# MIMUW-RL/space-gym

Measured on AMD Instinct MI355X. Metric: env-steps/sec at batch=65536, GoalContinuous3P-v0, 1/2/4/8 MI355X, higher is better.
Workload: dtype f32

## Files before the change

space_gym_amd/csrc/sg_device.hpp:

```cpp
#ifndef SG_DEVICE_HPP
#define SG_DEVICE_HPP

#include <math.h>
#include <stdint.h>

#include "sg_config.h"

#if defined(__HIPCC__)
#define SG_FN __device__ __forceinline__
#define SG_MFN __device__ __forceinline__
#else
#define SG_FN static inline
#define SG_MFN inline
#endif

#ifndef SG_STAMP
#define SG_STAMP(slot)
#endif

namespace sg {

#if defined(__HIP_DEVICE_COMPILE__)
SG_FN float rsq(float x) { return __builtin_amdgcn_rsqf(x); }
SG_FN float rcp(float x) { return __builtin_amdgcn_rcpf(x); }
// ... 925 lines not shown

SG_FN void tile_center(const SgDev &c, const Tiling &T, uint32_t tile, float &x, float &y) {
    uint32_t row = (tile * c.t_cols_rcp16) >> 16, col = tile - row * (uint32_t)c.t_cols;
    const float shift = (col == 1u) ? T.cs1 : (col == 2u) ? T.cs2 : (col == 3u) ? T.cs3 : T.cs0;
    float tx = c.t_x0 + (float)col * 1.5f * c.t_a + shift;
    float y0 = T.case_b ? c.t_y0 - 0.5f * c.t_hex_h : c.t_y0;
    float ycol = (col & 1u) ? 0.5f * c.t_hex_h : 0.0f;
    float ty = y0 - (float)row * c.t_hex_h + (T.case_b ? ycol : -ycol);
    x = T.flip ? ty : tx;
    y = T.flip ? tx : ty;
}

SG_FN void disc_in_tile(const SgDev &c, const Tiling &T, uint32_t tile, float noise_radius, uint32_t w, float &x, float &y) {
    float s, co;
    sincos_acc(kTwoPi * u16(w >> 16), s, co);
    float r = noise_radius * fsqrt(u16(w));
    tile_center(c, T, tile, x, y);
    x = fmaf(r, co, x);
    y = fmaf(r, s, y);
}

SG_FN void choose_goal_tile(const SgDev &c, Tiling &T, bool first, const uint32_t (&w)[4]) {
    if (!first) {
        T.free_counts = free_add(T.free_counts, T.ship_tile);
        T.ship_tile = T.goal_tile;
    }
    if ((w[0] & 0xffu) < 64u) {
        T.goal_tile = T.ship_tile;
    } else {
        const uint32_t n = free_total(T.free_counts), n_cand = n < 3u ? n : 3u;
        const uint32_t cols = (uint32_t)c.t_cols, sr = (T.ship_tile * c.t_cols_rcp16) >> 16, sc = T.ship_tile - sr * cols;
        const uint32_t draws[3] = {w[1] >> 16, w[1], w[2] >> 16};
        uint32_t chosen[3] = {0u, 0u, 0u};
        const uint32_t j0 = below16(draws[0], n);
        chosen[0] = j0;
        const uint32_t v1_old = (j0 == 1u) ? 0u : 1u;
        uint32_t j1 = 0xffffffffu;
        if (n_cand > 1) {
            j1 = 1u + below16(draws[1], n - 1u);
            chosen[1] = (j1 == j0) ? 0u : j1;
        }
        if (n_cand > 2) {
            const uint32_t j2 = 2u + below16(draws[2], n - 2u);
            chosen[2] = (j2 == j1) ? v1_old : (j2 == j0) ? 0u : j2;
        }
        uint32_t best_tile = 0;
        int best_dist = -1;
        const FreePrefix fp = free_prefix(T.free_counts);
#pragma unroll
        for (uint32_t i = 0; i < 3; i++) {
            if (i < n_cand) {
                uint32_t tile = free_at(fp, chosen[i]);
                uint32_t r = (tile * c.t_cols_rcp16) >> 16, cc = tile - r * cols;
                int dist = abs((int)r - (int)sr) + abs((int)cc - (int)sc);
                if (dist > best_dist) { best_dist = dist; best_tile = tile; }
            }
        }
        T.goal_tile = best_tile;
        T.free_counts = free_remove(T.free_counts, best_tile);
    }
}

SG_FN void choose_goal(const SgDev &c, Tiling &T, bool first, const uint32_t (&w)[4], float &gx, float &gy) {
    choose_goal_tile(c, T, first, w);
    disc_in_tile(c, T, T.goal_tile, c.noise_goal, w[3], gx, gy);
}

SG_FN void box_muller(uint32_t w1, uint32_t w2, float &z0, float &z1) {
    float r = fsqrt(-2.0f * 0.6931471805599453f * flog2(u23(w1)));
    float s, co;
    sincos_acc(kTwoPi * u23(w2), s, co);
    z0 = r * co;
    z1 = r * s;
}

struct ShipInit { float x, y, th, vx, vy, om; };

SG_FN void layout_from_words(const SgDev &c, uint32_t flags, uint32_t c01, uint32_t c23, Tiling &T) {
    T.case_b = flags & 1u; T.flip = (flags >> 1) & 1u;
    const float a0 = u16(c01 >> 16), a1 = a0 + u16(c01);
    const float a2 = (c.t_cols > 2) ? a1 + u16(c23 >> 16) : a1, a3 = (c.t_cols > 3) ? a2 + u16(c23) : a2;
    const float k = c.t_free_x * rcp(a3);
    T.cs0 = a0 * k; T.cs1 = a1 * k;
    T.cs2 = (c.t_cols > 2) ? a2 * k : 0.0f; T.cs3 = (c.t_cols > 3) ? a3 * k : 0.0f;
}

template <int N>
SG_FN void tiles_from_words(const SgDev &c, uint32_t flags, uint32_t t01, uint32_t t23, uint32_t t45, Tiling &T,
                            uint32_t (&tiles)[N + 1]) {
    const uint32_t draws[6] = {t01 >> 16, t01, t23 >> 16, t23, t45 >> 16, t45};
    uint64_t perm = 0xfedcba9876543210ull;
    const uint32_t nt = (uint32_t)c.t_tiles;
#pragma unroll
    for (uint32_t i = 0; i <= (uint32_t)N; i++) {
        uint32_t j = i + below16(draws[i], nt - i);
        uint64_t vi = (perm >> (4 * i)) & 15ull, vj = (perm >> (4 * j)) & 15ull;
        perm = (perm & ~((15ull << (4 * i)) | (15ull << (4 * j)))) | (vj << (4 * i)) | (vi << (4 * j));
        tiles[i] = (uint32_t)vj;
    }
    if (N == 2 && ((flags >> 8) & 0xffu) < 64u) {
        const uint32_t d = (flags >> 16) & 3u;
        tiles[0] = (d == 0) ? 1u : (d == 1) ? 2u : (d == 2) ? 0u : 3u;
        tiles[1] = (d < 2) ? 0u : 1u;
        tiles[2] = (d < 2) ? 3u : 2u;
    }
    uint64_t used = 0;
#pragma unroll
    for (int i = 0; i <= N; i++) used |= 1ull << (4 * tiles[i]);
    const uint64_t all = (nt >= 16u) ? 0x1111111111111111ull : (0x1111111111111111ull & ((1ull << (4 * nt)) - 1ull));
    T.free_counts = all & ~used;
    T.ship_tile = tiles[0];
}

SG_FN void kinematics_from_words(const SgDev &c, uint32_t wth, uint32_t b0, uint32_t b1, uint32_t b2, uint32_t b3, ShipInit &s) {
    s.th = kTwoPi * u23(wth);
    float z0, z1, z2, z3;
    box_muller(b0, b1, z0, z1);
    box_muller(b2, b3, z2, z3);
    s.vx = z0 * c.vel_std; s.vy = z1 * c.vel_std;
    s.om = fminf(fmaxf(z2 * c.omega_std, -c.omega_max), c.omega_max);
}

template <int N>
SG_FN void goal_reset(const SgDev &c, uint32_t env_global, Tiling &T, ShipInit &s, float (&px)[N], float (&py)[N],
                      float &gx, float &gy) {
    uint32_t w[4 * kGoalResetBlocks];
#pragma unroll
    for (uint32_t b = 0; b < (uint32_t)kGoalResetBlocks; b++) {
        uint32_t o[4];
        philox4x32_10(c.seed_lo, c.seed_hi, env_global, T.episode, b, kStreamReset, o);
        w[4 * b] = o[0]; w[4 * b + 1] = o[1]; w[4 * b + 2] = o[2]; w[4 * b + 3] = o[3];
    }
    T.goal_draws = 0;
    const uint32_t flags = w[0];
    layout_from_words(c, flags, w[1], w[2], T);
    uint32_t tiles[N + 1];
    tiles_from_words<N>(c, flags, w[3], w[4], w[5], T, tiles);
    disc_in_tile(c, T, tiles[0], c.noise_ship, w[8], s.x, s.y);
#pragma unroll
    for (int j = 0; j < N; j++) disc_in_tile(c, T, tiles[j + 1], c.noise_planet, w[9 + j], px[j], py[j]);
    const uint32_t gw[4] = {flags >> 24, w[6], w[7], w[13]};
    T.goal_tile = 0xffu;
    choose_goal(c, T, true, gw, gx, gy);
    kinematics_from_words(c, w[14], w[16], w[17], w[18], w[19], s);
}

SG_FN void goal_resample(const SgDev &c, uint32_t env_global, Tiling &T, float &gx, float &gy) {
    uint32_t w[4];
    T.goal_draws += 1;
    philox4x32_10(c.seed_lo, c.seed_hi, env_global, T.episode, T.goal_draws, kStreamGoal, w);
    choose_goal(c, T, false, w, gx, gy);
}

SG_FN void kepler_reset(const SgDev &c, uint32_t env_global, uint32_t episode, ShipInit &s, float &phi, float &ecc) {
    uint32_t w[4 * kKeplerResetBlocks];
#pragma unroll
    for (uint32_t b = 0; b < (uint32_t)kKeplerResetBlocks; b++) {
        uint32_t o[4];
        philox4x32_10(c.seed_lo, c.seed_hi, env_global, episode, b, kStreamReset, o);
        w[4 * b] = o[0]; w[4 * b + 1] = o[1]; w[4 * b + 2] = o[2]; w[4 * b + 3] = o[3];
    }
    float sa, ca;
    sincos_acc(kTwoPi * u23(w[0]), sa, ca);
    float dist = fmaf(c.kep_rmax - c.kep_rmin, u23(w[1]), c.kep_rmin);
    s.x = ca * dist; s.y = sa * dist;
    if (c.randomize_orbit) { ecc = u23(w[3]) * 0.7f; phi = u23(w[4]) * kTwoPi; }
    kinematics_from_words(c, w[2], w[8], w[9], w[10], w[11], s);
}

SG_FN void random_action_words(uint32_t seed_lo, uint32_t seed_hi, uint32_t env_global, uint64_t step, uint32_t &w0, uint32_t &w1) {
    uint32_t o[4];
    const uint64_t p = step >> 1;
    philox4x32_10(seed_lo, seed_hi, env_global, (uint32_t)p, (uint32_t)(p >> 32), kStreamAction, o);
    w0 = (step & 1u) ? o[2] : o[0];
    w1 = (step & 1u) ? o[3] : o[1];
}

template <int N>
struct GoalEnv {
    float x, y, th, vx, vy, om;
    float gx, gy;
    float px[N], py[N];
};
struct KeplerEnv {
    float x, y, th, vx, vy, om;
    float phi, ecc;
};

SG_FN void translate_action(float &a0, float &a1, float max_engine_force, float &engine, float &F, float &om) {
    a0 = fminf(fmaxf(a0, -1.0f), 1.0f);
    a1 = fminf(fmaxf(a1, -1.0f), 1.0f);
    engine = (a0 + 1.0f) * 0.5f;
    F = engine * max_engine_force;
    om = a1 * 5.0f;
}

template <bool ACCEL>
SG_FN void steering(const SgDev &c, float a1, float om_cmd, float om_state, float &om0, float &alpha) {
    if (ACCEL && c.steering_acceleration) { om0 = om_state; alpha = (a1 * c.max_thruster_force) * c.inv_moi; }
    else { om0 = om_cmd; alpha = 0.0f; }
}

SG_FN void load_action(bool discrete, const void *actions, int64_t idx, float &a0, float &a1) {
    if (discrete) {
        const int k = static_cast<const int32_t *>(actions)[idx];
        const bool engine = (k == 1) | (k == 4) | (k == 5);
        a0 = engine ? 1.0f : -1.0f;
        a1 = (k == 2 || k == 4) ? -1.0f : (k == 3 || k == 5) ? 1.0f : 0.0f;
    } else {
        const float *p = static_cast<const float *>(actions) + 2 * idx;
        a0 = p[0]; a1 = p[1];
    }
}

template <int N, typename CFG>
SG_FN void goal_observe(const CFG &c, const GoalEnv<N> &e, float (&obs)[7 + 2 * N + 2]) {
    float s, co;
    sincos_acc(e.th, s, co);
    obs[0] = e.x; obs[1] = e.y; obs[2] = co; obs[3] = s; obs[4] = e.vx; obs[5] = e.vy; obs[6] = e.om;
#pragma unroll
    for (int j = 0; j < N; j++) lidar(e.px[j] - e.x, e.py[j] - e.y, c.planet_r, c.two_over_world, obs[7 + 2 * j], obs[8 + 2 * j]);
    obs[7 + 2 * N] = (e.gx - e.x) * c.two_over_world;
    obs[8 + 2 * N] = (e.gy - e.y) * c.two_over_world;
}

template <typename CFG>
SG_FN void kepler_observe(const CFG &c, const KeplerEnv &e, float (&obs)[10]) {
    float s, co;
    sincos_acc(e.th, s, co);
    obs[0] = e.x; obs[1] = e.y; obs[2] = co; obs[3] = s; obs[4] = e.vx; obs[5] = e.vy; obs[6] = e.om;
    obs[7] = c.randomize_orbit ? e.phi : (float)c.k_phi;
    obs[8] = c.randomize_orbit ? e.ecc : (float)c.k_ecc;
    obs[9] = (float)c.k_a;
}

template <int N, bool ACCEL = false>
SG_FN void goal_env_begin(const SgDev &c, const GoalEnv<N> &e, float a0, float a1, Integrator<N, N, true, ACCEL> &I,
                          bool use_probe = true) {
    float engine, F, om, om0, alpha;
    translate_action(a0, a1, c.max_engine_force, engine, F, om);
    steering<ACCEL>(c, a1, om, e.om, om0, alpha);
    float cR[N];
    double cRd[N];
#pragma unroll
    for (int j = 0; j < N; j++) { cR[j] = c.planet_r; cRd[j] = c.planet_r_d; }
    I.begin(c.h, c.half_world, c.gm, F, om0, alpha, c.omega_limit, e.x, e.y, e.th, e.vx, e.vy, e.px, e.py, cR, cRd, use_probe);
}

struct GoalStepConsts {
    double goal_r2, danger_r2, survival, goal_scale, safety_scale, sparse;
    float planet_r, two_over_world;
};
SG_FN GoalStepConsts goal_step_consts(const SgDev &c) {
    GoalStepConsts k;
    k.goal_r2 = c.goal_r2; k.danger_r2 = c.danger_r2; k.survival = c.survival; k.goal_scale = c.goal_scale;
    k.safety_scale = c.safety_scale; k.sparse = c.sparse; k.planet_r = c.planet_r; k.two_over_world = c.two_over_world;
    return k;
}

struct KeplerStepConsts {
    double k_gm, k_C, k_Cr, k_phi, k_ecc, k_a;
    float k_Ca;
    int32_t randomize_orbit;
};
SG_FN KeplerStepConsts kepler_step_consts(const SgDev &c) {
    KeplerStepConsts k;
    k.k_gm = c.k_gm; k.k_C = c.k_C; k.k_Cr = c.k_Cr; k.k_phi = c.k_phi; k.k_ecc = c.k_ecc; k.k_a = c.k_a; k.k_Ca = c.k_Ca;
    k.randomize_orbit = c.randomize_orbit;
    return k;
}

struct GoalRewardProfile {
    double danger_r2, survival, goal_scale, safety_scale, sparse;
};
struct KeplerRewardProfile {
    double k_C, k_Cr;
    float k_Ca;
};
struct GoalRewardView {
    double goal_r2, danger_r2, survival, goal_scale, safety_scale, sparse;
};
SG_FN GoalRewardView goal_reward_view(const SgDev &c, const GoalRewardProfile &p) {
    GoalRewardView v;
    v.goal_r2 = c.goal_r2; v.danger_r2 = p.danger_r2; v.survival = p.survival; v.goal_scale = p.goal_scale;
    v.safety_scale = p.safety_scale; v.sparse = p.sparse;
    return v;
}
struct KeplerRewardView {
    double k_gm, k_C, k_Cr;
    float k_Ca;
};
SG_FN KeplerRewardView kepler_reward_view(const SgDev &c, const KeplerRewardProfile &p) {
    KeplerRewardView v;
    v.k_gm = c.k_gm; v.k_C = p.k_C; v.k_Cr = p.k_Cr; v.k_Ca = p.k_Ca;
    return v;
}

struct StepConsts {
    float max_engine_force, h, half_world, gm, omega_limit, planet_r, max_thruster_force, inv_moi;
    double planet_r_d;
    int32_t steering_acceleration;
};
SG_FN StepConsts step_consts(const SgDev &c) {
    StepConsts k;
    k.max_engine_force = c.max_engine_force; k.h = c.h; k.half_world = c.half_world; k.gm = c.gm; k.omega_limit = c.omega_limit;
    k.planet_r = c.planet_r; k.max_thruster_force = c.max_thruster_force; k.inv_moi = c.inv_moi; k.planet_r_d = c.planet_r_d;
// ... 98 lines not shown
```

space_gym_amd/csrc/sg_engine.hip:

```cpp
#include <hip/hip_runtime.h>
#include <hip/hip_ext.h>

#include <algorithm>
#include <array>
#include <cmath>
#include <cstdarg>
#include <cstdio>
#include <cstdlib>
#include <cstring>
#include <limits>
#include <new>
#include <string>
#include <tuple>
#include <type_traits>
#include <utility>
#include <vector>

#include "../../include/spacegym.h"

#ifdef SG_STAMPS
constexpr int kStampSlots = 16, kStampWaves = 4096;
__device__ unsigned long long sg_dbg_stamps[kStampSlots * kStampWaves];
#ifdef SG_STAMPS_ACC_ONLY
#define SG_STAMP(slot)
// ... 613 lines not shown
    using Env = GoalEnv<N>;
    using Rec = StepRecord<N>;
    using Integ = Integrator<N, N, true, ACCEL>;
    static constexpr int D = 7 + 2 * N + 2;
    static constexpr int kPre = 320, kWordsAt = 256;
    static constexpr bool kResample = true;
    static constexpr bool kTouchParams = true, kFinishAction = false;
    __device__ __forceinline__ explicit GoalStep(const SgDev &) {}
    __device__ __forceinline__ void load(const SgBuffers &b, int jj, float4 *base) const {
        __builtin_amdgcn_global_load_lds((gbl_void *)(b.pl[0] + jj), (lds_void *)(base + 128), 16, 0, 0);
        if constexpr (N > 2) __builtin_amdgcn_global_load_lds((gbl_void *)(b.pl[1] + jj), (lds_void *)(base + 192), 16, 0, 0);
    }
    __device__ __forceinline__ void read(const float4 *blk, int lane, Env &e) const {
        const float4 q0 = blk[lane], q1 = blk[64 + lane], p0 = blk[128 + lane];
        float4 p1 = {};
        if constexpr (N > 2) p1 = blk[192 + lane];
        e.x = q0.x; e.y = q0.y; e.th = q0.z; e.vx = q0.w;
        e.vy = q1.x; e.om = q1.y; e.gx = q1.z; e.gy = q1.w;
        e.px[0] = p0.x; e.py[0] = p0.y; e.px[1] = p0.z; e.py[1] = p0.w;
        if constexpr (N > 2) { e.px[2] = p1.x; e.py[2] = p1.y; }
        if constexpr (N > 3) { e.px[3] = p1.z; e.py[3] = p1.w; }
    }
    __device__ __forceinline__ static float2 q1_hi(const Env &e) { return make_float2(e.gx, e.gy); }
    __device__ __forceinline__ static int first(const SgDev &c, const Env &e, float2 a, StepResult &sr) {
        Integ I;
        goal_env_begin<N, ACCEL>(c, e, a.x, a.y, I);
        return I.first(sr, []() __attribute__((always_inline)) -> bool { return true; });
    }
    __device__ __forceinline__ static void integrate(const SgDev &c, const Env &e, float2 a, StepResult &sr) {
        Integ I;
        goal_env_begin<N, ACCEL>(c, e, a.x, a.y, I);
        I.run(sr);
    }
    __device__ __forceinline__ static void load_env(const SgBuffers &b, int i, Env &e) { load_goal_env<N>(b, i, e); }
    struct Ready {};
    __device__ __forceinline__ Ready load_finisher(const SgDev &, const SgBuffers &, int, const Env &) const { return {}; }
    __device__ __forceinline__ int pair_finish(const SgDev &c, const SgBuffers &b, Ready, Env &e, float2 a, const PairHand &h, bool live,
                                               float (&o)[D], float &r) const {
        return pair_finish_r(c, c, b, Ready{}, e, a, h, live, o, r);
    }
    template <typename RC>
    __device__ __forceinline__ static int pair_finish_r(const SgDev &c, const RC &rc, const SgBuffers &b, Ready, Env &e, float2,
                                                        const PairHand &h, bool live, float (&o)[D], float &r) {
        int hit;
        r = goal_reward<N>(rc, e.x, e.y, h.dXd, h.dYd, e.px, e.py, e.gx, e.gy, hit);
        e.x = (float)((double)e.x + h.dXd); e.y = (float)((double)e.y + h.dYd);
        e.th = h.th; e.vx = h.vx; e.vy = h.vy; e.om = h.om;
        goal_observe<N>(c, e, o);
        count_hits(b.cnt, live && hit);
        return hit;
    }
    __device__ __forceinline__ int finish(const SgDev &c, const SgBuffers &b, int, Env &e, float2, const StepResult &sr, bool kept,
                                          float (&o)[D], float &r) const {
        int dn, hit;
        goal_env_finish<N>(c, e, sr, o, r, dn, hit);
        count_hits(b.cnt, kept && hit);
        return hit;
    }
    template <typename RC>
    __device__ __forceinline__ static int finish_r(const SgDev &c, const RC &rc, const SgBuffers &b, Env &e, float2, const StepResult &sr,
                                                   bool kept, float (&o)[D], float &r) {
        int dn, hit;
        goal_env_finish_r<N>(c, rc, e, sr, o, r, dn, hit);
        count_hits(b.cnt, kept && hit);
        return hit;
    }
    __device__ __forceinline__ int replay(const SgDev &c, const SgBuffers &b, int, Env &e, float2 a, bool terminal, bool have,
                                          float (&o)[D], float &r, int &dn) const {
        StepResult r2;
        {
            Integ I;
            goal_env_begin<N, ACCEL>(c, e, a.x, a.y, I, false);
            I.run(r2);
        }
        if (terminal) r2.done = 1;
        int hit;
        goal_env_finish<N>(c, e, r2, o, r, dn, hit);
        count_hits(b.cnt, have && hit);
        return hit;
    }
    template <typename RC>
    __device__ __forceinline__ static int replay_r(const SgDev &c, const RC &rc, const SgBuffers &b, Env &e, float2 a, bool terminal,
                                                   bool have, float (&o)[D], float &r, int &dn) {
        StepResult r2;
        {
            Integ I;
            goal_env_begin<N, ACCEL>(c, e, a.x, a.y, I, false);
            I.run(r2);
        }
        if (terminal) r2.done = 1;
        int hit;
        goal_env_finish_r<N>(c, rc, e, r2, o, r, dn, hit);
        count_hits(b.cnt, have && hit);
        return hit;
    }
    struct Next {
        Tiling T;
        ShipInit s;
        float px[N], py[N], gx, gy;
    };
    __device__ __forceinline__ static float2 kept_orbit(const SgBuffers &, int) { return make_float2(0.0f, 0.0f); }
    __device__ __forceinline__ static float2 reset_orbit(const SgDev &) { return make_float2(0.0f, 0.0f); }
    __device__ __forceinline__ static void next(const SgDev &c, int env, uint32_t episode, float2, Next &n) {
        n.T.episode = episode;
        goal_reset<N>(c, c.env_index_base + (uint32_t)env, n.T, n.s, n.px, n.py, n.gx, n.gy);
    }
    __device__ __forceinline__ void install(const SgDev &c, const SgBuffers &b, int env, uint32_t episode, const Next &n, Env &e,
                                            float (&o)[D]) const {
        e.x = n.s.x; e.y = n.s.y; e.th = n.s.th; e.vx = n.s.vx; e.vy = n.s.vy; e.om = n.s.om; e.gx = n.gx; e.gy = n.gy;
#pragma unroll
        for (int j = 0; j < N; j++) { e.px[j] = n.px[j]; e.py[j] = n.py[j]; }
        store_goal_ship<N>(b, env, e);
        store_goal_planets<N>(b, env, e);
        store_tiling(b, env, n.T);
        b.ctr[env] = make_uint2(0u, episode);
        goal_observe<N>(c, e, o);
    }
    __device__ __forceinline__ static void empty_queue(const SgBuffers &b, int env, uint32_t episode) { b.ephi[env] = episode; }
    __device__ __forceinline__ static void restart_group(const SgDev &c, const SgBuffers &b, int env, uint32_t episode, int sub,
                                                         float *obs, float2) {
        Env ne;
        goal_restart_group<N>(c, b, env, episode, sub, obs, ne);
    }
    __device__ __forceinline__ static void resample(const SgDev &c, const SgBuffers &b, int env, uint32_t episode) {
        Tiling T = load_tiling(b, env, episode);
        float gx, gy;
        goal_resample(c, c.env_index_base + (uint32_t)env, T, gx, gy);
        reinterpret_cast<float2 *>(b.q1 + env)[1] = make_float2(gx, gy);
        b.aux[env] = pack_aux(T);
    }
    __device__ __forceinline__ static void resample_wave(const SgDev &c, const SgBuffers &b, int i, bool want, uint32_t episode) {
        const unsigned long long need = __ballot(want);
        if (!need) return;
        const int lane = threadIdx.x & 63, grp = lane >> 3, sub = lane & (kGroup - 1);
        const int n_items = __popcll(need), wave_env0 = i - lane;
        for (int base = 0; base < n_items; base += 64 / kGroup) {
            const int item = base + grp;
            const int src = nth_set_lane(need, item < n_items ? item : 0);
            const uint32_t ep = __shfl(episode, src);
            if (item < n_items && sub == 0) resample(c, b, wave_env0 + src, ep);
        }
    }
};

template <int N, bool ACCEL>
__global__ __launch_bounds__(kBlock) void goal_step_kernel(const SgDev *__restrict__ cfg, SgBuffers b, int n_subtiles,
                                                          const void *__restrict__ actions, float *__restrict__ obs,
                                                          float *__restrict__ reward, uint8_t *__restrict__ done,
                                                          uint8_t *__restrict__ truncated, float *__restrict__ terminal_obs,
                                                          int stream_out) {
    step_subtiles<GoalStep<N, ACCEL>>(cfg, b, n_subtiles, actions, obs, reward, done, truncated, terminal_obs, stream_out);
}

template <int N>
struct SpareEpisode {
    static constexpr int kFields = 6 + 2 * N + 2 + 7;
    __device__ __forceinline__ static void put(float *base, int slot, int tid, const ShipInit &s, const float (&px)[N],
                                               const float (&py)[N], float gx, float gy, const Tiling &T) {
        float *p = base + (slot * kFields) * kBlock + tid;
        int f = 0;
        auto w = [&](float v) { p[(f++) * kBlock] = v; };
        w(s.x); w(s.y); w(s.th); w(s.vx); w(s.vy); w(s.om); w(gx); w(gy);
#pragma unroll
        for (int j = 0; j < N; j++) { w(px[j]); w(py[j]); }
        const uint4 a = pack_aux(T);
        w(__uint_as_float(a.y)); w(__uint_as_float(a.z)); w(__uint_as_float(a.w));
        w(T.cs0); w(T.cs1); w(T.cs2); w(T.cs3);
    }
    __device__ __forceinline__ static void put_record(float *base, int slot, int tid, const float4 (&r)[6]) {
        float *p = base + (slot * kFields) * kBlock + tid;
        int f = 0;
        auto w = [&](float v) { p[(f++) * kBlock] = v; };
        w(r[0].x); w(r[0].y); w(r[0].z); w(r[0].w); w(r[1].x); w(r[1].y); w(r[1].z); w(r[1].w);
        w(r[2].x); w(r[2].y); w(r[2].z); w(r[2].w);
        if constexpr (N > 2) { w(r[3].x); w(r[3].y); }
        if constexpr (N > 3) { w(r[3].z); w(r[3].w); }
        w(r[4].x); w(r[4].y); w(r[4].z);
        w(r[5].x); w(r[5].y); w(r[5].z); w(r[5].w);
    }
    __device__ __forceinline__ static void get(const float *base, int slot, int tid, GoalEnv<N> &e, uint4 &aux, float4 &cs) {
        const float *p = base + (slot * kFields) * kBlock + tid;
        int f = 0;
        auto r = [&]() { return p[(f++) * kBlock]; };
        e.x = r(); e.y = r(); e.th = r(); e.vx = r(); e.vy = r(); e.om = r(); e.gx = r(); e.gy = r();
#pragma unroll
        for (int j = 0; j < N; j++) { e.px[j] = r(); e.py[j] = r(); }
        aux.x = 0u;
        aux.y = __float_as_uint(r()); aux.z = __float_as_uint(r()); aux.w = __float_as_uint(r());
        cs.x = r(); cs.y = r(); cs.z = r(); cs.w = r();
    }
};

template <int N, bool ACCEL, int kSpare>
__global__ __launch_bounds__(kBlock) __attribute__((amdgpu_waves_per_eu(2))) void goal_rollout_kernel(const SgDev *__restrict__ cfg, SgBuffers b, int n_steps,
                                                             const void *__restrict__ actions, float *__restrict__ obs,
                                                             float *__restrict__ reward, uint8_t *__restrict__ done,
                                                             uint8_t *__restrict__ truncated, TermList tl) {
    __shared__ float spare[kSpare * SpareEpisode<N>::kFields * kBlock];
    const SgDev &c = *cfg;
    const bool discrete = c.discrete_actions != 0;
    constexpr int D = 7 + 2 * N + 2;
    const int i = blockIdx.x * kBlock + threadIdx.x, tid = threadIdx.x;
    const bool live = i < c.num_envs;
    const int ii = live ? i : 0;
    const int64_t B = c.num_envs;
    GoalEnv<N> e;
    load_goal_env<N>(b, ii, e);
    uint2 ct = b.ctr[ii];
    int n_spare = 0;
    auto refill = [&]() {
        if (n_spare < kSpare) {
            Tiling T;
            T.episode = ct.y + (uint32_t)n_spare + 1u;
            ShipInit s;
            float px[N], py[N], gx, gy;
            goal_reset<N>(c, c.env_index_base + (uint32_t)ii, T, s, px, py, gx, gy);
            SpareEpisode<N>::put(spare, (int)(T.episode % (uint32_t)kSpare), tid, s, px, py, gx, gy, T);
            n_spare++;
        }
    };
    uint4 aux = b.aux[ii];
    float4 cs = b.cshift[ii];
    float2 a_next = load_action_raw(discrete, actions, ii);
    for (int t = 0; t < n_steps; t++) {
        const float2 a = decode_action(discrete, a_next);
        if (t + 1 < n_steps) a_next = load_action_raw(discrete, actions, (int64_t)(t + 1) * B + ii);
        StepResult sr;
        {
            Integrator<N, N, true, ACCEL> I;
            goal_env_begin<N, ACCEL>(c, e, a.x, a.y, I);
            I.run(sr);
        }
        float o[D], r;
        int hit;
        r = goal_reward<N>(c, e.x, e.y, sr.dXd, sr.dYd, e.px, e.py, e.gx, e.gy, hit);
        count_hits(b.cnt, live && hit);
        e.x = (float)((double)e.x + sr.dXd); e.y = (float)((double)e.y + sr.dYd); e.vx = sr.vx; e.vy = sr.vy; e.om = sr.om;
        e.th = wrap_two_pi(e.th + sr.dth);
        const uint32_t el = ct.x + 1u;
        const int trunc = !sr.done && (int)el >= c.max_episode_steps;
        const int fin = sr.done | trunc;
        const bool restart = live && fin && c.auto_reset;
        if (live) ct.x = el;
        if (tl.count && __any(restart)) {
            goal_observe<N>(c, e, o);
            term_append<D>(tl, restart, t, i, o);
        }
        if (__any(restart && n_spare == 0)) refill();
        if (restart) {
            ct = make_uint2(0u, ct.y + 1u);
            SpareEpisode<N>::get(spare, (int)(ct.y % (uint32_t)kSpare), tid, e, aux, cs);
            n_spare--;
        }
        goal_observe<N>(c, e, o);
        if (live) {
            const int64_t row = (int64_t)t * B + i;
            store_row(obs, row, o);
            reward[row] = r;
            done[row] = (uint8_t)fin;
            truncated[row] = (uint8_t)trunc;
        }
        if (live && hit && !restart) {
            Tiling T;
            T.episode = ct.y; T.goal_draws = aux.x;
            T.ship_tile = aux.y & 0xffu; T.goal_tile = (aux.y >> 8) & 0xffu; T.case_b = (aux.y >> 16) & 1u; T.flip = (aux.y >> 17) & 1u;
            T.free_counts = (uint64_t)aux.z | ((uint64_t)aux.w << 32);
            T.cs0 = cs.x; T.cs1 = cs.y; T.cs2 = cs.z; T.cs3 = cs.w;
            goal_resample(c, c.env_index_base + (uint32_t)i, T, e.gx, e.gy);
            aux = pack_aux(T);
        }
    }
    if (live) {
        store_goal_ship<N>(b, i, e);
        store_goal_planets<N>(b, i, e);
        b.ctr[i] = ct;
        b.aux[i] = aux;
        b.cshift[i] = cs;
    }
}

constexpr int kPairBlock = 2 * kBlock;
#ifndef SG_RING
#define SG_RING 5
#endif
constexpr int kRing = SG_RING;
constexpr int kHand = 9;
constexpr int kReplayCap = 128;
#ifndef SG_REPLAY_AT
#define SG_REPLAY_AT 56
#endif
#ifndef SG_PILOT_SLEEP
#define SG_PILOT_SLEEP 40
#endif
constexpr int kReplayAt = SG_REPLAY_AT;
constexpr uint32_t kSpinLimit = 1u << 21;

constexpr int kQDepth = 4;
constexpr int kQCols = 6;
template <int N>
struct EpisodeQueue {
    __device__ __forceinline__ static float4 *slot(float4 *q, int64_t B, int i, uint32_t episode) {
        return q + ((episode % (uint32_t)kQDepth) * (uint32_t)kQCols * (uint32_t)B + (uint32_t)i);
    }
    __device__ __forceinline__ static void put(float4 *q, int64_t B, int i, const ShipInit &s, const float (&px)[N],
                                               const float (&py)[N], float gx, float gy, const Tiling &T) {
        float4 *p = slot(q, B, i, T.episode);
        p[0] = make_float4(s.x, s.y, s.th, s.vx);
        p[B] = make_float4(s.vy, s.om, gx, gy);
        p[2 * B] = make_float4(px[0], py[0], px[1], py[1]);
        if constexpr (N == 3) p[3 * B] = make_float4(px[2], py[2], 0.0f, 0.0f);
        if constexpr (N == 4) p[3 * B] = make_float4(px[2], py[2], px[3], py[3]);
        const uint4 a = pack_aux(T);
        p[4 * B] = make_float4(__uint_as_float(a.y), __uint_as_float(a.z), __uint_as_float(a.w), 0.0f);
        p[5 * B] = make_float4(T.cs0, T.cs1, T.cs2, T.cs3);
    }
};

__device__ __forceinline__ uint32_t flag_load(const uint32_t *p) {
    return __hip_atomic_load(p, __ATOMIC_ACQUIRE, __HIP_MEMORY_SCOPE_WORKGROUP);
}
__device__ __forceinline__ void flag_store(uint32_t *p, uint32_t v) {
    __hip_atomic_store(p, v, __ATOMIC_RELEASE, __HIP_MEMORY_SCOPE_WORKGROUP);
}
__device__ __forceinline__ uint32_t lds_flag_load(const uint32_t *p) {
    const uint32_t v = __hip_atomic_load(p, __ATOMIC_RELAXED, __HIP_MEMORY_SCOPE_WORKGROUP);
    __builtin_amdgcn_fence(__ATOMIC_ACQUIRE, "workgroup", "local");
    return v;
}
__device__ __forceinline__ uint32_t lds_flag_peek(const uint32_t *p) {
    return __hip_atomic_load(p, __ATOMIC_RELAXED, __HIP_MEMORY_SCOPE_WORKGROUP);
}
__device__ __forceinline__ void lds_flag_store(uint32_t *p, uint32_t v) {
    __builtin_amdgcn_fence(__ATOMIC_RELEASE, "workgroup", "local");
    __hip_atomic_store(p, v, __ATOMIC_RELAXED, __HIP_MEMORY_SCOPE_WORKGROUP);
}
__device__ __forceinline__ uint32_t lds_flag_load_uniform(const uint32_t *p) {
    return (uint32_t)__builtin_amdgcn_readfirstlane((int)lds_flag_load(p));
}
template <int kSleep = 1>
__device__ __forceinline__ bool wait_flag(const uint32_t *flag, uint32_t want, uint32_t *seen = nullptr) {
    uint32_t v = lds_flag_load_uniform(flag);
    if ((int32_t)(v - want) < 0) {
#pragma unroll 1
        for (uint32_t n = 0; n < kSpinLimit; n++) {
            __builtin_amdgcn_s_sleep(kSleep);
            v = lds_flag_load_uniform(flag);
            if ((int32_t)(v - want) >= 0) break;
        }
        if ((int32_t)(v - want) < 0) return false;
    }
    if (seen) *seen = v;
    return true;
}

template <int N>
struct GoalReplay {
    static constexpr int kWords = 13 + 2 * N;
    __device__ __forceinline__ static void put(float *rb, uint32_t slot, uint32_t step_lane, const GoalEnv<N> &e, float2 a) {
        float *q = rb + slot;
        int f = 0;
        auto w = [&](float v) { q[(f++) * kReplayCap] = v; };
        w(__uint_as_float(step_lane));
        w(e.x); w(e.y); w(e.th); w(e.vx); w(e.vy); w(e.om); w(a.x); w(a.y);
#pragma unroll
        for (int j = 0; j < N; j++) { w(e.px[j]); w(e.py[j]); }
    }
    __device__ __forceinline__ static void put_goal(float *rb, uint32_t slot, float gx, float gy) {
        rb[(9 + 2 * N) * kReplayCap + slot] = gx; rb[(10 + 2 * N) * kReplayCap + slot] = gy;
    }
    __device__ __forceinline__ static void get(const float *rb, uint32_t slot, uint32_t &step_lane, GoalEnv<N> &e, float2 &a) {
        const float *q = rb + slot;
        int f = 0;
        auto r = [&]() { return q[(f++) * kReplayCap]; };
        step_lane = __float_as_uint(r());
        e.x = r(); e.y = r(); e.th = r(); e.vx = r(); e.vy = r(); e.om = r(); a.x = r(); a.y = r();
#pragma unroll
        for (int j = 0; j < N; j++) { e.px[j] = r(); e.py[j] = r(); }
        e.gx = r(); e.gy = r();
    }
    __device__ __forceinline__ static void put_result(float *rb, uint32_t slot, const StepResult &r, float th) {
        float *q = rb + slot;
        const uint64_t ux = __double_as_longlong(r.dXd), uy = __double_as_longlong(r.dYd);
        q[3 * kReplayCap] = th; q[4 * kReplayCap] = r.vx; q[5 * kReplayCap] = r.vy; q[6 * kReplayCap] = r.om;
        q[7 * kReplayCap] = __uint_as_float((uint32_t)ux); q[8 * kReplayCap] = __uint_as_float((uint32_t)(ux >> 32));
        q[(11 + 2 * N) * kReplayCap] = __uint_as_float((uint32_t)uy); q[(12 + 2 * N) * kReplayCap] = __uint_as_float((uint32_t)(uy >> 32));
    }
    __device__ __forceinline__ static void get_result(const float *rb, uint32_t slot, double &dXd, double &dYd) {
        const float *q = rb + slot;
        const uint64_t ux = (uint64_t)__float_as_uint(q[7 * kReplayCap]) | ((uint64_t)__float_as_uint(q[8 * kReplayCap]) << 32);
        const uint64_t uy = (uint64_t)__float_as_uint(q[(11 + 2 * N) * kReplayCap]) | ((uint64_t)__float_as_uint(q[(12 + 2 * N) * kReplayCap]) << 32);
        dXd = __longlong_as_double((long long)ux); dYd = __longlong_as_double((long long)uy);
    }
};

struct NoTermList {};
struct NoProfileSource {
    static constexpr bool kOn = false;
};
struct ProfileSource {
    static constexpr bool kOn = true;
    const void *table;
    const uint8_t *idx;
    __device__ __forceinline__ GoalRewardView goal(const SgDev &c, int env) const {
        return goal_reward_view(c, static_cast<const GoalRewardProfile *>(table)[idx[env]]);
    }
    __device__ __forceinline__ KeplerRewardView kepler(const SgDev &c, int env) const {
        return kepler_reward_view(c, static_cast<const KeplerRewardProfile *>(table)[idx[env]]);
    }
};

template <int N, bool ACCEL, bool TOBS, typename TL, typename RS = NoProfileSource>
__device__ __forceinline__ void goal_replay_pass(const SgDev &c, const float *rb, uint32_t lo, uint32_t n, int lane, int wave_env0,
                                                 int64_t B, float *__restrict__ reward, const TL &tl, uint32_t *tail,
                                                 unsigned long long *cnt, const RS &rs = RS{}) {
    constexpr int D = 7 + 2 * N + 2;
    const bool have = (uint32_t)lane < n;
    const uint32_t slot = (lo + (have ? (uint32_t)lane : 0u)) % (uint32_t)kReplayCap;
    uint32_t step_lane;
    GoalEnv<N> e;
    float2 a;
    GoalReplay<N>::get(rb, slot, step_lane, e, a);
    lds_flag_store(tail, lo + n);
    StepResult r;
    {
        Integrator<N, N, true, ACCEL> I;
        goal_env_begin<N, ACCEL>(c, e, a.x, a.y, I, false);
        I.run(r);
    }
    int hit;
    float rew;
    if constexpr (RS::kOn) rew = goal_reward<N>(rs.goal(c, wave_env0 + (int)(step_lane & 63u)), e.x, e.y, r.dXd, r.dYd, e.px, e.py, e.gx, e.gy, hit);
    else rew = goal_reward<N>(c, e.x, e.y, r.dXd, r.dYd, e.px, e.py, e.gx, e.gy, hit);
    count_hits(cnt, have && hit);
    const int t = (int)(step_lane >> 6), env = wave_env0 + (int)(step_lane & 63u);
    if (have) reward[(int64_t)t * B + env] = rew;
    if constexpr (TOBS) {
        e.x = (float)((double)e.x + r.dXd); e.y = (float)((double)e.y + r.dYd); e.vx = r.vx; e.vy = r.vy; e.om = r.om;
        e.th = wrap_two_pi(e.th + r.dth);
        float o[D];
        goal_observe<N>(c, e, o);
        term_append<D>(tl, have, t, env, o);
    }
}

template <int N, bool ACCEL>
__device__ __forceinline__ void goal_replay_integrate(const SgDev &c, float *rb, uint32_t lo, uint32_t n, int lane) {
    const bool have = (uint32_t)lane < n;
    const uint32_t slot = (lo + (have ? (uint32_t)lane : 0u)) % (uint32_t)kReplayCap;
    uint32_t step_lane;
    GoalEnv<N> e;
    float2 a;
    GoalReplay<N>::get(rb, slot, step_lane, e, a);
    StepResult r;
    {
        Integrator<N, N, true, ACCEL> I;
        goal_env_begin<N, ACCEL>(c, e, a.x, a.y, I, false);
        I.run(r);
    }
    if (have) GoalReplay<N>::put_result(rb, slot, r, wrap_two_pi(e.th + r.dth));
}
template <int N, bool TOBS, typename TL, typename RS = NoProfileSource>
__device__ __forceinline__ void goal_replay_reward(const SgDev &c, const float *rb, uint32_t lo, uint32_t n, int lane, int wave_env0,
                                                   int64_t B, float *__restrict__ reward, const TL &tl, unsigned long long *cnt,
                                                   const RS &rs = RS{}) {
    constexpr int D = 7 + 2 * N + 2;
    const bool have = (uint32_t)lane < n;
    const uint32_t slot = (lo + (have ? (uint32_t)lane : 0u)) % (uint32_t)kReplayCap;
    uint32_t step_lane;
    GoalEnv<N> e;
// ... 5074 lines not shown
```

space_gym_amd/csrc/sg_goal_pair_rollout.inc:

```

    const SgBuffers &b = *bufs;
    using Spare = SpareEpisode<N>;
    using Queue = EpisodeQueue<N>;
    using Integ = Integrator<N, N, true, ACCEL>;
    using Replay = GoalReplay<N>;
    __shared__ float spare[kSpare * Spare::kFields * kBlock];
    __shared__ float ring[kRing * kHand * kBlock];
    __shared__ float rbuf[(kBlock / 64) * Replay::kWords * kReplayCap];
    __shared__ uint32_t spare_hi[kBlock];
    __shared__ uint32_t handed[kBlock / 64], taken[kBlock / 64];
    __shared__ uint32_t rp_tail[kBlock / 64];
    __shared__ uint32_t rp_claim[kBlock / 64], rp_done[kBlock / 64];
    constexpr int D = 7 + 2 * N + 2;
    SG_REAL(0);
    const int tid = threadIdx.x & (kBlock - 1), pair = tid >> 6, lane = tid & 63;
    const bool pilot = threadIdx.x < kBlock;
    const int i = blockIdx.x * kBlock + tid;
    const bool live = i < num_envs;
    const int ii = live ? i : 0;
    const int64_t B = num_envs;
    GoalEnv<N> e;
    load_goal_env<N>(b, ii, e);
    uint2 ct = b.ctr[ii];
    const SgDev &c = *cfg;
    {
        const uint32_t *cw = reinterpret_cast<const uint32_t *>(cfg);
        uint32_t touch = 0u;
#pragma unroll
        for (int k = 0; k < (int)(sizeof(SgDev) / 4); k += 16) touch ^= cw[k];
        touch ^= cw[sizeof(SgDev) / 4 - 1];
        asm volatile("" ::"s"(touch));
    }
    const bool discrete = c.discrete_actions != 0;
    float *const rb = rbuf + pair * Replay::kWords * kReplayCap;
    if (!pilot) spare_hi[tid] = ct.y;
    if (threadIdx.x < kBlock / 64) { handed[threadIdx.x] = 0u; taken[threadIdx.x] = 0u; rp_tail[threadIdx.x] = 0u; rp_claim[threadIdx.x] = 0u; rp_done[threadIdx.x] = 0u; }
    __syncthreads();
    SG_REAL(1);

    if (pilot) {
        SG_ACC_DECL;
        __builtin_amdgcn_s_setprio(3);
        const bool hand_over = c.auto_reset && live;
        const bool auto_reset = c.auto_reset != 0;
        StepConsts kc = step_consts(c);
        asm volatile("" : "+v"(kc.max_engine_force), "+v"(kc.h), "+v"(kc.half_world), "+v"(kc.gm), "+v"(kc.omega_limit), "+v"(kc.planet_r),
                          "+v"(kc.max_thruster_force), "+v"(kc.inv_moi), "+v"(kc.planet_r_d));
        int max_steps = c.max_episode_steps;
        asm volatile("" : "+v"(max_steps));
        float2 a_next = load_action_raw(discrete, actions, ii);
        uint32_t taken_seen = 0u;
        uint32_t head = 0u, tail_seen = 0u;
        for (int t = 0; t < n_steps; t++) {
            const float2 a = decode_action(discrete, a_next);
            if (t + 1 < n_steps) a_next = load_action_raw(discrete, actions, (int64_t)(t + 1) * B + ii);
            if (t - (int)taken_seen >= kRing && !wait_flag<SG_PILOT_SLEEP>(&taken[pair], (uint32_t)(t - kRing + 1), &taken_seen)) { *status = 1; break; }
            if (head + 64u - tail_seen > (uint32_t)kReplayCap) tail_seen = lds_flag_load_uniform(&rp_tail[pair]);
            const bool defer = hand_over && head + 64u - tail_seen <= (uint32_t)kReplayCap;

            const int slot = t % kRing;
            StepResult r;
            int rk;
            {
                Integ I;
                SG_ACC(0);
                goal_env_begin<N, ACCEL>(kc, e, a.x, a.y, I);
                SG_ACC(1);
                rk = I.run(r, [&]() __attribute__((always_inline)) -> bool { return defer; });
                SG_ACC_ADD(7, __any(r.done) ? 1 : 0);
                SG_ACC_ADD(10, __any(r.path == kPathScipyErr || r.path == kPathScipyClear) ? 1 : 0);
                SG_ACC_ADD(11, __any((r.path == kPathScipyErr || r.path == kPathScipyClear) && r.n_rk > 1) ? 1 : 0);
                SG_ACC(2);
            }
            const bool replayed = rk == kRkEventDeferred;
            uint32_t rslot = 0u;
            {
                const unsigned long long dm = __ballot(replayed);
                if (dm) {
                    rslot = (head + (uint32_t)__popcll(dm & ((1ull << lane) - 1ull))) % (uint32_t)kReplayCap;
                    if (replayed) Replay::put(rb, rslot, ((uint32_t)t << 6) | (uint32_t)lane, e, a);
                    head += (uint32_t)__popcll(dm);
                }
            }
            e.x = (float)((double)e.x + r.dXd); e.y = (float)((double)e.y + r.dYd); e.vx = r.vx; e.vy = r.vy; e.om = r.om;
            e.th = wrap_two_pi(e.th + r.dth);
            SG_ACC(3);
            SG_ACC(4);
            {
                float *q = ring + (slot * kHand) * kBlock + tid;
                const uint64_t ux = __double_as_longlong(r.dXd), uy = __double_as_longlong(r.dYd);
                q[0 * kBlock] = __uint_as_float((uint32_t)ux); q[1 * kBlock] = __uint_as_float((uint32_t)(ux >> 32));
                q[2 * kBlock] = __uint_as_float((uint32_t)uy); q[3 * kBlock] = __uint_as_float((uint32_t)(uy >> 32));
                q[4 * kBlock] = e.th; q[5 * kBlock] = e.vx; q[6 * kBlock] = e.vy; q[7 * kBlock] = e.om;
                q[8 * kBlock] = __uint_as_float((uint32_t)r.done | (replayed ? 2u | (rslot << 8) : 0u));
            }
            lds_flag_store(&handed[pair], (uint32_t)(t + 1));
            SG_ACC(5);
            const uint32_t el = ct.x + 1u;
            const int trunc = !r.done && (int)el >= max_steps;
            const bool restart = live && (r.done | trunc) && auto_reset;
            if (live) ct.x = el;
            if (restart) {
                const uint32_t k = ct.y + 1u;
                if ((int32_t)(lds_flag_load(&spare_hi[tid]) - k) >= 0) {
                    const float *q = spare + ((int)(k % (uint32_t)kSpare) * Spare::kFields) * kBlock + tid;
                    e.x = q[0 * kBlock]; e.y = q[1 * kBlock]; e.th = q[2 * kBlock]; e.vx = q[3 * kBlock];
                    e.vy = q[4 * kBlock]; e.om = q[5 * kBlock];
#pragma unroll
                    for (int j = 0; j < N; j++) { e.px[j] = q[(8 + 2 * j) * kBlock]; e.py[j] = q[(9 + 2 * j) * kBlock]; }
                } else {
                    Tiling T;
                    T.episode = k;
                    ShipInit s;
                    float gx, gy;
                    goal_reset<N>(c, c.env_index_base + (uint32_t)i, T, s, e.px, e.py, gx, gy);
                    e.x = s.x; e.y = s.y; e.th = s.th; e.vx = s.vx; e.vy = s.vy; e.om = s.om;
                }
                ct = make_uint2(0u, k);
            }
            SG_ACC(8);
        }
        SG_ACC_WRITE(blockIdx.x * 8 + pair);
        SG_REAL(2);
        if (live) {
            b.q0[i] = make_float4(e.x, e.y, e.th, e.vx);
            reinterpret_cast<float2 *>(b.q1 + i)[0] = make_float2(e.vy, e.om);
            store_goal_planets<N>(b, i, e);
            b.ctr[i] = ct;
        }
        {
            uint32_t lo = 0u;
            if (lane == 0) lo = atomicMax(&rp_claim[pair], head);
            lo = (uint32_t)__builtin_amdgcn_readfirstlane((int)lo);
            __builtin_amdgcn_fence(__ATOMIC_SEQ_CST, "wavefront");
#pragma unroll 1
            while ((int32_t)(head - lo) > 0) {
                const uint32_t n = min(head - lo, 64u);
                goal_replay_integrate<N, ACCEL>(c, rb, lo, n, lane);
                lo += n;
            }
            lds_flag_store(&rp_done[pair], 1u);
        }
        SG_REAL(3);
        return;
    }

    SG_ACC_DECL;
    const bool auto_reset = c.auto_reset != 0;
    const int wave_env0 = i - lane;
    unsigned long long *const cnt = b.cnt;
    GoalStepConsts fc = goal_step_consts(c);
#if SG_ROLLOUT_PROFILED
    {
        const GoalRewardView v = rs.goal(c, ii);
        fc.danger_r2 = v.danger_r2; fc.survival = v.survival; fc.goal_scale = v.goal_scale; fc.safety_scale = v.safety_scale;
        fc.sparse = v.sparse;
    }
#endif
    asm volatile("" : "+v"(fc.goal_r2), "+v"(fc.danger_r2), "+v"(fc.survival), "+v"(fc.goal_scale), "+v"(fc.safety_scale),
                      "+v"(fc.sparse), "+v"(fc.planet_r), "+v"(fc.two_over_world));
    int max_steps = c.max_episode_steps;
    asm volatile("" : "+v"(max_steps));
    uint32_t hi = ct.y;
    uint4 aux = b.aux[ii];
    float4 cs = b.cshift[ii];
    if (auto_reset) {
        const uint32_t q_hi = b.ephi[ii];
        const int n_have = live ? min(max((int32_t)(q_hi - ct.y), 0), kSpare) : 0;
        float4 rec[kSpare][kQCols];
#pragma unroll
        for (int s = 0; s < kSpare; s++)
            if (s < n_have) {
                const float4 *p = Queue::slot(b.epq, B, i, ct.y + 1u + (uint32_t)s);
#pragma unroll
                for (int col = 0; col < kQCols; col++)
                    if (col != 3 || N > 2) rec[s][col] = p[(uint32_t)col * (uint32_t)B];
            }
#pragma unroll
        for (int s = 0; s < kSpare; s++)
            if (s < n_have) Spare::put_record(spare, (int)((ct.y + 1u + (uint32_t)s) % (uint32_t)kSpare), tid, rec[s]);
        hi = ct.y + (uint32_t)n_have;
        lds_flag_store(&spare_hi[tid], hi);
    }
    auto refill = [&]() {
        SG_ACC_ADD(10, 1);
        if (live && hi - ct.y < (uint32_t)kSpare) {
            Tiling T;
            T.episode = hi + 1u;
            ShipInit s;
            float px[N], py[N], gx, gy;
            goal_reset<N>(c, c.env_index_base + (uint32_t)i, T, s, px, py, gx, gy);
            Spare::put(spare, (int)(T.episode % (uint32_t)kSpare), tid, s, px, py, gx, gy, T);
            Queue::put(b.epq, B, i, s, px, py, gx, gy, T);
            hi = T.episode;
            lds_flag_store(&spare_hi[tid], hi);
        }
    };
    constexpr uint32_t kKeep = 1u;
    if (auto_reset && __any(live && hi - ct.y < kKeep)) refill();
    uint32_t tail = 0u, complete = 0u;
    bool mine = true;
    typedef __attribute__((address_space(1))) float gfloat;
    typedef __attribute__((address_space(1))) uint8_t gbyte;
    gfloat *obs_p = (gfloat *)obs + (int64_t)ii * D, *rew_p = (gfloat *)reward + ii;
    gbyte *done_p = (gbyte *)done + ii, *trunc_p = (gbyte *)truncated + ii;
    asm volatile("" : "+v"(obs_p), "+v"(rew_p), "+v"(done_p), "+v"(trunc_p));
    for (int t = 0; t < n_steps; t++) {
        SG_ACC(0);
        if (!wait_flag(&handed[pair], (uint32_t)(t + 1))) { *status = 2; break; }
        SG_ACC(1);
        double dXd, dYd;
        float th, vx, vy, om;
        int dn;
        bool replayed;
        {
            const int slot = t % kRing;
            const float *q = ring + (slot * kHand) * kBlock + tid;
            const uint64_t ux = (uint64_t)__float_as_uint(q[0 * kBlock]) | ((uint64_t)__float_as_uint(q[1 * kBlock]) << 32);
            const uint64_t uy = (uint64_t)__float_as_uint(q[2 * kBlock]) | ((uint64_t)__float_as_uint(q[3 * kBlock]) << 32);
            dXd = __longlong_as_double((long long)ux); dYd = __longlong_as_double((long long)uy);
            th = q[4 * kBlock]; vx = q[5 * kBlock]; vy = q[6 * kBlock]; om = q[7 * kBlock];
            const uint32_t w8 = __float_as_uint(q[8 * kBlock]);
            dn = (int)(w8 & 1u);
            replayed = (w8 & 2u) != 0u;
            if (replayed) Replay::put_goal(rb, w8 >> 8, e.gx, e.gy);
            complete += (uint32_t)__popcll(__ballot(replayed));
        }
        lds_flag_store(&taken[pair], (uint32_t)(t + 1));
        SG_ACC(3);
        float o[D], r;
        int hit;
        r = goal_reward<N>(fc, e.x, e.y, dXd, dYd, e.px, e.py, e.gx, e.gy, hit);
        count_hits(cnt, live && hit && !replayed);
        e.x = (float)((double)e.x + dXd); e.y = (float)((double)e.y + dYd); e.vx = vx; e.vy = vy; e.om = om; e.th = th;
        const uint32_t el = ct.x + 1u;
        const int trunc = !dn && (int)el >= max_steps;
        const int fin = dn | trunc;
        const bool restart = live && fin && auto_reset;
        if (live) ct.x = el;
        SG_ACC(4);
        if constexpr (TOBS) {
            if (__any(restart && !replayed)) {
                goal_observe<N>(fc, e, o);
                term_append<D>(tl, restart && !replayed, t, i, o);
            }
        }
        const uint32_t keep = t + 1 < n_steps ? kKeep : 0u;
        if (auto_reset && __any(live && hi - ct.y < (restart ? keep + 1u : keep))) refill();
        SG_ACC(6);
        if (restart) {
            ct = make_uint2(0u, ct.y + 1u);
            Spare::get(spare, (int)(ct.y % (uint32_t)kSpare), tid, e, aux, cs);
        }
        SG_ACC(12);
        goal_observe<N>(fc, e, o);
        SG_ACC(13);
        if (live) {
#pragma unroll
            for (int k = 0; k < D; k++) obs_p[k] = o[k];
            if (!replayed) *rew_p = r;
            *done_p = (uint8_t)fin;
            *trunc_p = (uint8_t)trunc;
        }
        obs_p += B * D; rew_p += B; done_p += B; trunc_p += B;
        asm volatile("" : "+v"(obs_p), "+v"(rew_p), "+v"(done_p), "+v"(trunc_p));
        SG_ACC(5);
        SG_ACC(7);
        SG_ACC_ADD(11, __any(live && hit && !restart) ? 1 : 0);
        if (live && hit && !restart) {
            Tiling T;
            T.episode = ct.y; T.goal_draws = aux.x;
            T.ship_tile = aux.y & 0xffu; T.goal_tile = (aux.y >> 8) & 0xffu; T.case_b = (aux.y >> 16) & 1u; T.flip = (aux.y >> 17) & 1u;
            T.free_counts = (uint64_t)aux.z | ((uint64_t)aux.w << 32);
            T.cs0 = cs.x; T.cs1 = cs.y; T.cs2 = cs.z; T.cs3 = cs.w;
            goal_resample(c, c.env_index_base + (uint32_t)i, T, e.gx, e.gy);
            aux = pack_aux(T);
        }
        SG_ACC(2);
        if (complete - tail >= (uint32_t)kReplayAt && mine) {
            const uint32_t n = min(complete - tail, 64u);
            uint32_t got = 0u;
            if (lane == 0) got = atomicCAS(&rp_claim[pair], tail, tail + n);
            mine = (uint32_t)__builtin_amdgcn_readfirstlane((int)got) == tail;
            if (mine) {
                __builtin_amdgcn_fence(__ATOMIC_ACQ_REL, "workgroup", "local");
                goal_replay_pass<N, ACCEL, TOBS>(c, rb, tail, n, lane, wave_env0, B, reward, tl, &rp_tail[pair], cnt SG_ROLLOUT_RS);
                tail += n;
            }
        }
        SG_ACC(9);
    }
    SG_ACC_WRITE(blockIdx.x * 8 + 4 + pair);
    SG_REAL(2);
    if (live) {
        reinterpret_cast<float2 *>(b.q1 + i)[1] = make_float2(e.gx, e.gy);
        b.aux[i] = aux;
        b.cshift[i] = cs;
        if (auto_reset) b.ephi[i] = hi;
    }
    if (tail != complete) {
        if (!wait_flag(&rp_done[pair], 1u)) *status = 3;
#pragma unroll 1
        while (tail != complete) {
            const uint32_t n = min(complete - tail, 64u);
            goal_replay_reward<N, TOBS>(c, rb, tail, n, lane, wave_env0, B, reward, tl, cnt SG_ROLLOUT_RS);
            tail += n;
        }
    }
    SG_REAL(3);
```

Baseline: 29.23 billion.

## Precompute first goal resample at episode reset and apply it on goal hit

When a spare episode is generated during refill, the first goal resample is also computed and stored with it: the next goal position and the packed tile bits go into the spare LDS slot and into the HBM episode queue record. When the ship reaches its first goal, the step loop applies this stored goal through a few bit operations instead of running the philox plus choose_goal resample in the divergent hot loop. The cost is more LDS per spare slot, extra work at refill time, and tile-state bookkeeping that must match the original resample exactly. It is enabled by default for N=3 only.

```diff
diff --git a/space_gym_amd/csrc/sg_device.hpp b/space_gym_amd/csrc/sg_device.hpp
--- a/space_gym_amd/csrc/sg_device.hpp
+++ b/space_gym_amd/csrc/sg_device.hpp
@@ -1101,6 +1101,30 @@
     choose_goal(c, T, false, w, gx, gy);
 }
 
+constexpr uint32_t kTilesMask = 0x3ffffu;
+constexpr uint32_t kNextTileShift = 18u, kNextKept = 1u << 26, kNextValid = 1u << 27;
+SG_FN uint32_t next_goal_pack(uint32_t tiles, uint32_t tile, bool kept) {
+    return (tiles & kTilesMask) | ((tile & 0xffu) << kNextTileShift) | (kept ? kNextKept : 0u) | kNextValid;
+}
+SG_FN uint32_t next_goal_tiles(uint32_t word) { return word & kTilesMask; }
+SG_FN uint32_t next_goal_bits(uint32_t word) { return word & ~kTilesMask; }
+SG_FN uint32_t next_goal_tile(uint32_t word) { return (word >> kNextTileShift) & 0xffu; }
+SG_FN uint32_t next_goal_generate(const SgDev &c, uint32_t env_global, const Tiling &T0, float &gx1, float &gy1) {
+    Tiling T = T0;
+    gx1 = 0.0f; gy1 = 0.0f;
+    goal_resample(c, env_global, T, gx1, gy1);
+    const bool kept = T.free_counts == free_add(T0.free_counts, T0.ship_tile);
+    return next_goal_bits(next_goal_pack(0u, T.goal_tile, kept));
+}
+SG_FN void next_goal_apply(Tiling &T, uint32_t bits) {
+    const uint32_t tile = next_goal_tile(bits);
+    T.goal_draws = 1u;
+    T.free_counts = free_add(T.free_counts, T.ship_tile);
+    T.ship_tile = T.goal_tile;
+    T.goal_tile = tile;
+    if (!(bits & kNextKept)) T.free_counts = free_remove(T.free_counts, tile);
+}
+
 SG_FN void kepler_reset(const SgDev &c, uint32_t env_global, uint32_t episode, ShipInit &s, float &phi, float &ecc) {
     uint32_t w[4 * kKeplerResetBlocks];
 #pragma unroll
diff --git a/space_gym_amd/csrc/sg_engine.hip b/space_gym_amd/csrc/sg_engine.hip
--- a/space_gym_amd/csrc/sg_engine.hip
+++ b/space_gym_amd/csrc/sg_engine.hip
@@ -789,11 +789,12 @@
     step_subtiles<GoalStep<N, ACCEL>>(cfg, b, n_subtiles, actions, obs, reward, done, truncated, terminal_obs, stream_out);
 }
 
-template <int N>
+template <int N, bool NEXT = false>
 struct SpareEpisode {
-    static constexpr int kFields = 6 + 2 * N + 2 + 7;
+    static constexpr int kFields = 6 + 2 * N + 2 + 7 + (NEXT ? 2 : 0);
     __device__ __forceinline__ static void put(float *base, int slot, int tid, const ShipInit &s, const float (&px)[N],
-                                               const float (&py)[N], float gx, float gy, const Tiling &T) {
+                                               const float (&py)[N], float gx, float gy, const Tiling &T,
+                                               uint32_t next_bits = 0u, float gx1 = 0.0f, float gy1 = 0.0f) {
         float *p = base + (slot * kFields) * kBlock + tid;
         int f = 0;
         auto w = [&](float v) { p[(f++) * kBlock] = v; };
@@ -801,8 +802,9 @@
 #pragma unroll
         for (int j = 0; j < N; j++) { w(px[j]); w(py[j]); }
         const uint4 a = pack_aux(T);
-        w(__uint_as_float(a.y)); w(__uint_as_float(a.z)); w(__uint_as_float(a.w));
+        w(__uint_as_float(NEXT ? a.y | next_bits : a.y)); w(__uint_as_float(a.z)); w(__uint_as_float(a.w));
         w(T.cs0); w(T.cs1); w(T.cs2); w(T.cs3);
+        if constexpr (NEXT) { w(gx1); w(gy1); }
     }
     __device__ __forceinline__ static void put_record(float *base, int slot, int tid, const float4 (&r)[6]) {
         float *p = base + (slot * kFields) * kBlock + tid;
@@ -814,8 +816,10 @@
         if constexpr (N > 3) { w(r[3].z); w(r[3].w); }
         w(r[4].x); w(r[4].y); w(r[4].z);
         w(r[5].x); w(r[5].y); w(r[5].z); w(r[5].w);
+        if constexpr (NEXT) { static_assert(!NEXT || N == 3, "the HBM record has room for the next goal at N = 3 only"); w(r[3].z); w(r[3].w); }
     }
     __device__ __forceinline__ static void get(const float *base, int slot, int tid, GoalEnv<N> &e, uint4 &aux, float4 &cs) {
+        static_assert(!NEXT, "with NEXT the record's next goal is taken too");
         const float *p = base + (slot * kFields) * kBlock + tid;
         int f = 0;
         auto r = [&]() { return p[(f++) * kBlock]; };
@@ -825,6 +829,21 @@
         aux.x = 0u;
         aux.y = __float_as_uint(r()); aux.z = __float_as_uint(r()); aux.w = __float_as_uint(r());
         cs.x = r(); cs.y = r(); cs.z = r(); cs.w = r();
+    }
+    __device__ __forceinline__ static void get(const float *base, int slot, int tid, GoalEnv<N> &e, uint4 &aux, float4 &cs,
+                                               uint32_t &next_bits, float &gx1, float &gy1) {
+        const float *p = base + (slot * kFields) * kBlock + tid;
+        int f = 0;
+        auto r = [&]() { return p[(f++) * kBlock]; };
+        e.x = r(); e.y = r(); e.th = r(); e.vx = r(); e.vy = r(); e.om = r(); e.gx = r(); e.gy = r();
+#pragma unroll
+        for (int j = 0; j < N; j++) { e.px[j] = r(); e.py[j] = r(); }
+        aux.x = 0u;
+        const uint32_t word = __float_as_uint(r());
+        aux.y = next_goal_tiles(word); next_bits = next_goal_bits(word);
+        aux.z = __float_as_uint(r()); aux.w = __float_as_uint(r());
+        cs.x = r(); cs.y = r(); cs.z = r(); cs.w = r();
+        gx1 = r(); gy1 = r();
     }
 };
 
@@ -951,7 +970,25 @@
         p[4 * B] = make_float4(__uint_as_float(a.y), __uint_as_float(a.z), __uint_as_float(a.w), 0.0f);
         p[5 * B] = make_float4(T.cs0, T.cs1, T.cs2, T.cs3);
     }
+    __device__ __forceinline__ static void put(float4 *q, int64_t B, int i, const ShipInit &s, const float (&px)[N],
+                                               const float (&py)[N], float gx, float gy, const Tiling &T, uint32_t next_bits,
+                                               float gx1, float gy1) {
+        static_assert(N == 3, "no room in the record at other N");
+        float4 *p = slot(q, B, i, T.episode);
+        p[0] = make_float4(s.x, s.y, s.th, s.vx);
+        p[B] = make_float4(s.vy, s.om, gx, gy);
+        p[2 * B] = make_float4(px[0], py[0], px[1], py[1]);
+        p[3 * B] = make_float4(px[2], py[2], gx1, gy1);
+        const uint4 a = pack_aux(T);
+        p[4 * B] = make_float4(__uint_as_float(a.y | next_bits), __uint_as_float(a.z), __uint_as_float(a.w), 0.0f);
+        p[5 * B] = make_float4(T.cs0, T.cs1, T.cs2, T.cs3);
+    }
 };
+#ifndef SG_NEXT_GOAL
+#define SG_NEXT_GOAL 1
+#endif
+template <int N>
+constexpr bool kNextGoal = SG_NEXT_GOAL != 0 && N == 3;
 
 __device__ __forceinline__ uint32_t flag_load(const uint32_t *p) {
     return __hip_atomic_load(p, __ATOMIC_ACQUIRE, __HIP_MEMORY_SCOPE_WORKGROUP);
diff --git a/space_gym_amd/csrc/sg_goal_pair_rollout.inc b/space_gym_amd/csrc/sg_goal_pair_rollout.inc
--- a/space_gym_amd/csrc/sg_goal_pair_rollout.inc
+++ b/space_gym_amd/csrc/sg_goal_pair_rollout.inc
@@ -1,6 +1,7 @@
 
     const SgBuffers &b = *bufs;
-    using Spare = SpareEpisode<N>;
+    constexpr bool NEXT = kNextGoal<N>;
+    using Spare = SpareEpisode<N, NEXT>;
     using Queue = EpisodeQueue<N>;
     using Integ = Integrator<N, N, true, ACCEL>;
     using Replay = GoalReplay<N>;
@@ -11,6 +12,8 @@
     __shared__ uint32_t handed[kBlock / 64], taken[kBlock / 64];
     __shared__ uint32_t rp_tail[kBlock / 64];
     __shared__ uint32_t rp_claim[kBlock / 64], rp_done[kBlock / 64];
+    static_assert(sizeof(spare) + sizeof(ring) + sizeof(rbuf) + sizeof(spare_hi) + sizeof(handed) + sizeof(taken) + sizeof(rp_tail) +
+                      sizeof(rp_claim) + sizeof(rp_done) <= 160u * 1024u, "the kernel's static LDS must fit one workgroup per CU");
     constexpr int D = 7 + 2 * N + 2;
     SG_REAL(0);
     const int tid = threadIdx.x & (kBlock - 1), pair = tid >> 6, lane = tid & 63;
@@ -164,6 +167,8 @@
     uint32_t hi = ct.y;
     uint4 aux = b.aux[ii];
     float4 cs = b.cshift[ii];
+    uint32_t next_bits = 0u;
+    float next_gx = 0.0f, next_gy = 0.0f;
     if (auto_reset) {
         const uint32_t q_hi = b.ephi[ii];
         const int n_have = live ? min(max((int32_t)(q_hi - ct.y), 0), kSpare) : 0;
@@ -190,8 +195,15 @@
             ShipInit s;
             float px[N], py[N], gx, gy;
             goal_reset<N>(c, c.env_index_base + (uint32_t)i, T, s, px, py, gx, gy);
-            Spare::put(spare, (int)(T.episode % (uint32_t)kSpare), tid, s, px, py, gx, gy, T);
-            Queue::put(b.epq, B, i, s, px, py, gx, gy, T);
+            if constexpr (NEXT) {
+                float gx1, gy1;
+                const uint32_t nb = next_goal_generate(c, c.env_index_base + (uint32_t)i, T, gx1, gy1);
+                Spare::put(spare, (int)(T.episode % (uint32_t)kSpare), tid, s, px, py, gx, gy, T, nb, gx1, gy1);
+                Queue::put(b.epq, B, i, s, px, py, gx, gy, T, nb, gx1, gy1);
+            } else {
+                Spare::put(spare, (int)(T.episode % (uint32_t)kSpare), tid, s, px, py, gx, gy, T);
+                Queue::put(b.epq, B, i, s, px, py, gx, gy, T);
+            }
             hi = T.episode;
             lds_flag_store(&spare_hi[tid], hi);
         }
@@ -250,7 +262,8 @@
         SG_ACC(6);
         if (restart) {
             ct = make_uint2(0u, ct.y + 1u);
-            Spare::get(spare, (int)(ct.y % (uint32_t)kSpare), tid, e, aux, cs);
+            if constexpr (NEXT) Spare::get(spare, (int)(ct.y % (uint32_t)kSpare), tid, e, aux, cs, next_bits, next_gx, next_gy);
+            else Spare::get(spare, (int)(ct.y % (uint32_t)kSpare), tid, e, aux, cs);
         }
         SG_ACC(12);
         goal_observe<N>(fc, e, o);
@@ -266,8 +279,25 @@
         asm volatile("" : "+v"(obs_p), "+v"(rew_p), "+v"(done_p), "+v"(trunc_p));
         SG_ACC(5);
         SG_ACC(7);
-        SG_ACC_ADD(11, __any(live && hit && !restart) ? 1 : 0);
-        if (live && hit && !restart) {
+        bool resample = live && hit && !restart;
+        if constexpr (NEXT) {
+            const bool take = resample && aux.x == 0u && (next_bits & kNextValid) != 0u;
+            SG_ACC_ADD(14, __any(take) ? 1 : 0);
+            if (take) {
+                Tiling T;
+                T.ship_tile = aux.y & 0xffu; T.goal_tile = (aux.y >> 8) & 0xffu;
+                T.free_counts = (uint64_t)aux.z | ((uint64_t)aux.w << 32);
+                next_goal_apply(T, next_bits);
+                aux.x = T.goal_draws;
+                aux.y = (aux.y & ~0xffffu) | T.ship_tile | (T.goal_tile << 8);
+                aux.z = (uint32_t)T.free_counts; aux.w = (uint32_t)(T.free_counts >> 32);
+                e.gx = next_gx; e.gy = next_gy;
+                next_bits = 0u;
+            }
+            resample = resample && !take;
+        }
+        SG_ACC_ADD(11, __any(resample) ? 1 : 0);
+        if ((!NEXT || __any(resample)) && resample) {
             Tiling T;
             T.episode = ct.y; T.goal_draws = aux.x;
             T.ship_tile = aux.y & 0xffu; T.goal_tile = (aux.y >> 8) & 0xffu; T.case_b = (aux.y >> 16) & 1u; T.flip = (aux.y >> 17) & 1u;
```

Result: no change. 29.38 billion, median of 6 (+0.5%).
